# Zeudon/sound-event-localization-detection

Hardware: AMD Instinct MI355X
Metric: training clips/sec (4ch FOA 60s@24kHz) (higher is better)
Workload: dtype bf16; 1 GPU; crnn FOA 4-ch 60s clips, bs=32 windows (BASELINE configs[1]); parallelism=dp1

## Files before the change

include/seld_hip.h:

```cpp
#ifndef SELD_HIP_H_
#define SELD_HIP_H_

#include <stdint.h>

#ifdef __cplusplus
extern "C" {
#endif

int seld_init(int device);
int seld_shutdown(void);
int seld_version(void);
const char* seld_last_error(void);

int seld_set_mel_filterbank(const float* fb_host);

int seld_set_window(const float* window_host);

int seld_default_tables(float* window960, float* fb481x64, int* mel_b0_64, float* mel_wd_24x64,
                        float* mel_wu_24x64);

int64_t seld_num_frames(int64_t L);

int seld_logmel_f32(const float* pcm, int64_t N, int64_t C, int64_t L, float* out, int layout, void* stream);
int seld_logmel_i16(const int16_t* pcm, int64_t N, int64_t C, int64_t L, float* out, int layout, void* stream);
// ... 106 lines not shown
                  float* loss_out4, void* grad, void* workspace, void* stream);


int seld_gru_fold_bias(const float* b_ih, const float* b_hh, int64_t H, void* gi_bias, int out_is_bf16, float* b_hn,
                       void* stream);

int seld_gru_prepare(const float* b_ih, const float* b_hh, const void* w_hh, int w_is_bf16, int64_t H, void* gi_bias,
                     int out_is_bf16, float* b_hn, void* w_hh_t_bf16, void* stream);

int seld_gru_bias_grads(const float* partial, int64_t tiles, int64_t H, float* db_ih, float* db_hh, void* stream);

int seld_sum_chunks(const void* partial, int in_is_bf16, int64_t chunks, int64_t count, void* out, int out_is_bf16,
                    void* stream);

int64_t seld_column_sums_blocks(int64_t rows, int64_t n_cols);
int seld_column_sums(const void* g, int in_is_bf16, int64_t rows, int64_t n_cols, float* partial, void* out, int out_is_bf16,
                     void* stream);

int seld_multi_sum_chunks(const void* const* partial, void* const* out, const int64_t* counts, const int32_t* chunks,
                          const int32_t* flags, int count, void* stream);
int seld_multi_column_sums_scratch(const int64_t* rows, const int64_t* n_cols, int count, int64_t* partial_floats);
int seld_multi_column_sums(const void* const* g, void* const* out, const int64_t* rows, const int64_t* n_cols,
                           const int32_t* flags, int count, float* partial, int64_t partial_floats, void* stream);

int seld_gru_dwhh_finish(const void* p_gi, const void* p_n, int in_is_bf16, int64_t chunks, int64_t H, void* dw_hh,
                         int out_is_bf16, void* stream);

int seld_conv_weight_flip_transpose(const void* w, int elem_bytes, int64_t O, int64_t I, void* wt, void* stream);

int seld_conv3x3_wgrad_supported(int64_t F, int64_t Cin, int64_t Cout);
int64_t seld_conv3x3_wgrad_workspace_floats(int64_t B, int64_t T, int64_t F, int64_t Cin, int64_t Cout);
int seld_conv3x3_wgrad(const void* x, const void* dy, int64_t B, int64_t T, int64_t F, int64_t Cin, int64_t Cout,
                       void* dw, int dw_is_bf16, float* workspace, void* stream);

int seld_convfirst_supported(int64_t F, int64_t Cin, int64_t Cout);
int64_t seld_convfirst_workspace_floats(int backward);
int seld_convfirst_forward(const void* in, const void* w, int w_is_bf16, int64_t w_sco, int64_t w_sci, int64_t w_sr,
                           int64_t w_ss, int64_t B, int64_t T, int64_t F, const float* bn_weight, const float* bn_bias,
                           float* running_mean, float* running_var, float momentum, float eps, void* y,
                           float* mean_invstd, float* scale_shift, float* workspace, int phases, void* stream);
int seld_convfirst_backward(const void* in, const void* w, int w_is_bf16, int64_t w_sco, int64_t w_sci, int64_t w_sr,
                            int64_t w_ss, const void* dy, int64_t B, int64_t T, int64_t F, const float* mean_invstd,
                            const float* scale_shift, void* dw, int dw_is_bf16, int64_t dw_sco, int64_t dw_sci,
                            int64_t dw_sr, int64_t dw_ss, float* dgamma, float* dbeta, float* workspace, int phases,
                            void* stream);

int64_t seld_conv_tail_workspace_floats(int C);
int seld_conv_tail_forward(const void* x, const void* residual, int is_bf16, int64_t rows, int C, int pool,
                           const float* weight, const float* bias, float* running_mean, float* running_var,
                           float momentum, float eps, int training, void* y, float* mean_invstd, float* scale_shift,
                           float* workspace, void* stream);
int seld_conv_tail_backward(const void* x, const void* residual, const void* dy, int is_bf16, int64_t rows, int C,
                            int pool, const float* mean_invstd, const float* scale_shift, void* dx, void* dresidual,
                            float* dweight, float* dbias, float* workspace, void* stream);

int seld_dwconv1d(const void* x, int is_bf16, const float* weight, const float* bias, int64_t B, int64_t T, int D, int K,
                  int flip_taps, void* y, void* stream);
int64_t seld_dwconv1d_wgrad_rows(int64_t B, int64_t T);
int seld_dwconv1d_wgrad(const void* x, const void* dy, int is_bf16, int64_t B, int64_t T, int D, int K, float* partial,
                        void* stream);

int64_t seld_gru_tile_rows(void);
int seld_gru_forward(const void* gi, int is_bf16, const void* w_hh_bf16, const float* b_hn, int64_t B,
                     int64_t T, int64_t H, void* y, void* saved_tile, void* stream);

int seld_gru_backward(const void* dy_tile, const void* saved_tile, const void* y, int is_bf16,
// ... 36 lines not shown
```

sound-event-localization-detection_amd/config.py:

```python
from pathlib import Path

_SR = 24000


class Config:
    BASE_PATH = Path(__file__).parent
    AUDIO_PATH = BASE_PATH / "foa_dev"
    METADATA_PATH = BASE_PATH / "metadata_dev"
    OUTPUT_PATH = BASE_PATH / "outputs"
    CHECKPOINT_PATH = BASE_PATH / "checkpoints"

    USE_FULL_DATASET = True
    TRAIN_AUDIO_FILE = "fold3_room21_mix001.wav"
    TRAIN_META_FILE = "fold3_room21_mix001.csv"
    TEST_AUDIO_FILE = "fold4_room23_mix001.wav"
    TEST_META_FILE = "fold4_room23_mix001.csv"

    STARSS22_CLASSES = dict(enumerate((
        "Female speech, woman speaking", "Male speech, man speaking", "Clapping", "Telephone",
        "Laughter", "Domestic sounds", "Walk, footsteps", "Door, open or close", "Music",
        "Musical instrument", "Water tap, faucet", "Bell", "Knock", "Background")))

    MODEL_TYPE = "resnet_conformer"
    NUM_CLASSES = 14
# ... 21 lines not shown
    LR_DECAY_FACTOR = 0.5
    LR_DECAY_PATIENCE = 5
    WEIGHT_DECAY = 1e-4

    LOSS_TYPE = "mse"
    W_CLASS = 1.0
    W_AIUR = 1.0
    W_CL = 1.0

    PATIENCE = 20
    MIN_DELTA = 1e-4

    SAVE_EVERY_N_EPOCHS = 5
    KEEP_LAST_N_CHECKPOINTS = 3

    SPECTROGRAM_N_FFT = int(0.04 * _SR)
    SPECTROGRAM_HOP_LENGTH = int(0.02 * _SR)
    N_MELS = 64
    SR = _SR

    WINDOW_LENGTH = int(5 * _SR)
    HOP_LENGTH = int(1 * _SR)

    I = None
    J = None
    GRID_CELL_DEGREES = 10

    AMP_DTYPE = "bf16"
    CHANNELS_LAST = True
    FUSED_LOSS = True
    FUSED_CONV_TAIL = True
    CONV_DGRAD_AS_FORWARD = True
    FUSED_CONV_WGRAD = True
    FUSED_FIRST_BLOCK = True
    FUSED_DWCONV = "auto"
    CONV1X1_AS_GEMM = True
    FUSED_QKV = True
    FUSED_LAYERNORM = True
    OVERLAP_WEIGHT_GRADS = True
    FUSED_GRU = True
    DEVICE_FEED = True
    MASTER_WEIGHTS = True
    FUSED_ADAM_KERNEL = True
    GRAPH_STEP = True
    OVERLAP_ALLREDUCE = True
    ALLREDUCE_CUT_LEVELS = 2
    GRAD_REDUCE_DTYPE = "param"
    TUNED_GEMMS = True
    DDP_BUCKET_MB = 8
    SYNC_BATCHNORM = False
    SEED = None
    FEATURE_SET = "logmel"
    FEATURE_CACHE_DIR = None
    THREE_TERM_LOSS = False
    GAUSSIAN_AUGMENT = False
    GAUSSIAN_SIGMA_AZIMUTH = 5.0
    GAUSSIAN_SIGMA_ELEVATION = 5.0
    AUGMENT_SPATIAL = False
    AUGMENT_TIME_MASKS = 0
    AUGMENT_TIME_MASK_MAX = 0
    AUGMENT_FREQ_MASKS = 0
    AUGMENT_FREQ_MASK_MAX = 0
    AUGMENT_MASK_VALUE = 0.0
    FOA_CHANNEL_ORDER = "WYZX"
    GRAD_CLIP_NORM = 0.0
    SKIP_NONFINITE_STEPS = False
# ... 25 lines not shown
```

sound-event-localization-detection_amd/csrc/convwgrad.hip:

```cpp
#include <hip/hip_bf16.h>

#include "seld_common.h"

namespace seld {

namespace {

typedef __attribute__((ext_vector_type(8))) __bf16 bf16x8;
typedef __attribute__((ext_vector_type(4))) short s16x4;
typedef __attribute__((ext_vector_type(8))) short s16x8;
typedef __attribute__((ext_vector_type(4))) float f32x4;
typedef __attribute__((address_space(3))) s16x4 lds_s16x4;

constexpr int kWgThreads = 256;
constexpr int kWgTile = 64;
constexpr int kWgKc = 128;
constexpr int kWgPitch = 80;
constexpr int kWgSumThreads = 256;
constexpr int kWgSumRows = 8;

template <int F>
struct WgradGeom {
  static_assert(F == 8 || F == 16 || F == 32, "frequency bins: 8, 16 or 32");
  static constexpr int TC = kWgKc / F;
  static constexpr int XR = (TC + 2) * (F + 2);
  static constexpr int kDyLoads = kWgKc * 8 / kWgThreads;
  static constexpr int kXLoads = (XR * 8 + kWgThreads - 1) / kWgThreads;
  static constexpr int kLdsShorts = (kWgKc + XR) * kWgPitch;
  static_assert(kLdsShorts * 2 <= 64 * 1024, "LDS image larger than the default limit");
};

template <int F>
__device__ __forceinline__ int x_row(int pos) {
  return (pos / F + 1) * (F + 2) + pos % F + 1;
}

__device__ __forceinline__ s16x4 tr_read(const unsigned short* base, int offset_shorts) {
  return __builtin_amdgcn_ds_read_tr16_b64_v4i16((lds_s16x4*)(base + offset_shorts));
}

__device__ __forceinline__ bf16x8 join(s16x4 lo, s16x4 hi) {
  const s16x8 v = __builtin_shufflevector(lo, hi, 0, 1, 2, 3, 4, 5, 6, 7);
  return __builtin_bit_cast(bf16x8, v);
}

template <int F>
__global__ __launch_bounds__(kWgThreads, 2) void conv3x3_wgrad_kernel(
    const unsigned short* __restrict__ x, const unsigned short* __restrict__ dy, int T, int Cin, int Cout,
    int chunks_per_clip, int chunks, int per_slab, float* __restrict__ ws) {
  using G = WgradGeom<F>;
  __shared__ __attribute__((aligned(16))) unsigned short lds[G::kLdsShorts];
  unsigned short* const ldy = lds;
  unsigned short* const lx = lds + kWgKc * kWgPitch;

  const int tid = threadIdx.x, lane = tid & 63, wave = tid >> 6;
  const int wm = wave >> 1, wn = wave & 1;
  const int ci0 = blockIdx.x * kWgTile, co0 = blockIdx.y * kWgTile;
  const int c_begin = blockIdx.z * per_slab;
  const int c_end = min(c_begin + per_slab, chunks);

  f32x4 acc[9][2][2];
#pragma unroll
  for (int k = 0; k < 9; ++k)
#pragma unroll
    for (int m = 0; m < 2; ++m)
#pragma unroll
      for (int n = 0; n < 2; ++n) acc[k][m][n] = f32x4{0.0f, 0.0f, 0.0f, 0.0f};

  const int g = lane >> 4, q = (lane >> 2) & 3, p = lane & 3;
  const int lpos = 4 * g + q;
  const int a_col = wm * 32 + 4 * p, b_col = wn * 32 + 4 * p;

  uint4 rdy[G::kDyLoads], rx[G::kXLoads];
  auto load = [&](int c) {
    const int b = c / chunks_per_clip, t0 = (c - b * chunks_per_clip) * G::TC;
    const long clip_row = static_cast<long>(b) * T;
#pragma unroll
    for (int i = 0; i < G::kDyLoads; ++i) {
      const int piece = tid + i * kWgThreads, pos = piece >> 3, ch = piece & 7;
      const int t = t0 + pos / F;
      rdy[i] = make_uint4(0u, 0u, 0u, 0u);
      if (t < T)
        rdy[i] = *reinterpret_cast<const uint4*>(dy + ((clip_row + t) * F + pos % F) * Cout + co0 + ch * 8);
    }
#pragma unroll
    for (int i = 0; i < G::kXLoads; ++i) {
      const int piece = tid + i * kWgThreads, r = piece >> 3, ch = piece & 7;
      const int tr = r / (F + 2), f = r - tr * (F + 2) - 1, t = t0 - 1 + tr;
      rx[i] = make_uint4(0u, 0u, 0u, 0u);
      if (r < G::XR && t >= 0 && t < T && f >= 0 && f < F)
        rx[i] = *reinterpret_cast<const uint4*>(x + ((clip_row + t) * F + f) * Cin + ci0 + ch * 8);
    }
  };

  for (int c = c_begin; c < c_end; ++c) {
    load(c);
    __syncthreads();
#pragma unroll
    for (int i = 0; i < G::kDyLoads; ++i) {
      const int piece = tid + i * kWgThreads;
      *reinterpret_cast<uint4*>(ldy + (piece >> 3) * kWgPitch + (piece & 7) * 8) = rdy[i];
    }
#pragma unroll
    for (int i = 0; i < G::kXLoads; ++i) {
      const int piece = tid + i * kWgThreads;
      if (piece < G::XR * 8) *reinterpret_cast<uint4*>(lx + (piece >> 3) * kWgPitch + (piece & 7) * 8) = rx[i];
    }
    __syncthreads();

#pragma unroll
    for (int ks = 0; ks < kWgKc / 32; ++ks) {
      const int pos_lo = ks * 32 + lpos, pos_hi = pos_lo + 16;
      bf16x8 a[2];
#pragma unroll
      for (int m = 0; m < 2; ++m)
        a[m] = join(tr_read(ldy, pos_lo * kWgPitch + a_col + m * 16), tr_read(ldy, pos_hi * kWgPitch + a_col + m * 16));
      const int xr_lo = x_row<F>(pos_lo), xr_hi = x_row<F>(pos_hi);
#pragma unroll
      for (int tap = 0; tap < 9; ++tap) {
        const int shift = (tap / 3 - 1) * (F + 2) + (tap % 3 - 1);
        bf16x8 bfr[2];
#pragma unroll
        for (int n = 0; n < 2; ++n)
          bfr[n] = join(tr_read(lx, (xr_lo + shift) * kWgPitch + b_col + n * 16),
                        tr_read(lx, (xr_hi + shift) * kWgPitch + b_col + n * 16));
#pragma unroll
        for (int m = 0; m < 2; ++m)
#pragma unroll
          for (int n = 0; n < 2; ++n)
            acc[tap][m][n] = __builtin_amdgcn_mfma_f32_16x16x32_bf16(a[m], bfr[n], acc[tap][m][n], 0, 0, 0);
      }
    }
  }

  float* const slot = ws + static_cast<long>(blockIdx.z) * Cout * 9 * Cin;
#pragma unroll
  for (int m = 0; m < 2; ++m)
#pragma unroll
    for (int j = 0; j < 4; ++j) {
      const int co = co0 + wm * 32 + m * 16 + 4 * (lane >> 4) + j;
#pragma unroll
      for (int tap = 0; tap < 9; ++tap)
#pragma unroll
        for (int n = 0; n < 2; ++n)
          slot[(static_cast<long>(co) * 9 + tap) * Cin + ci0 + wn * 32 + n * 16 + (lane & 15)] = acc[tap][m][n][j];
    }
}

template <bool kBf16>
__global__ __launch_bounds__(kWgSumThreads) void conv3x3_wgrad_sum_kernel(const float* __restrict__ ws, int slabs,
                                                                           long count, void* __restrict__ dw) {
  constexpr int kCols = kWgSumThreads / kWgSumRows;
  __shared__ float4 part[kWgSumRows][kCols];
// ... 115 lines not shown
```

sound-event-localization-detection_amd/model_crnn.py:

```python
import torch
import torch.nn as nn
import torch.nn.functional as F

from seld_layernorm import run_head
from seld_linear import SeldLinear
from seld_rnn import SeldGRU


class _Conv3x3(torch.autograd.Function):

    enabled = True
    fused_wgrad = True

    @staticmethod
    def forward(ctx, x, weight):
        cdt = torch.get_autocast_dtype("cuda") if torch.is_autocast_enabled() else x.dtype
        with torch.autocast(device_type="cuda", enabled=False):
            xc, wc = x.to(cdt), weight.to(cdt)
            y = F.conv2d(xc, wc, padding=1)
        ctx.save_for_backward(xc, wc)
        ctx.dtypes = (x.dtype, weight.dtype)
        ctx.after_cut = bool(x.is_leaf and x.requires_grad)
        return y

    @staticmethod
    def backward(ctx, dy):
        xc, wc = ctx.saved_tensors
        x_dtype, w_dtype = ctx.dtypes
        with torch.autocast(device_type="cuda", enabled=False):
            dy = dy.to(xc.dtype).contiguous(memory_format=torch.channels_last)
            dx = None
            if ctx.needs_input_grad[0]:
                if wc.is_contiguous(memory_format=torch.channels_last):
                    import seld_native
                    wt = seld_native.conv_weight_flip_transpose(wc)
                else:
                    wt = wc.transpose(0, 1).flip(2, 3).contiguous(memory_format=torch.channels_last)
                import seld_overlap
                seld_overlap.release_held(dy.device)
                dx = F.conv2d(dy, wt, padding=1)
                if dx.dtype != x_dtype:
                    dx = dx.to(x_dtype)
            import seld_overlap
            import seld_native
            fused = _Conv3x3.fused_wgrad and seld_native.conv3x3_wgrad_applicable(xc, dy, wc)
            if seld_overlap.conv_wgrad_side and seld_overlap.enabled:
                dw = torch.empty_like(wc, dtype=w_dtype)

                def job():
                    if fused:
                        seld_native.conv3x3_wgrad(xc, dy, dw)
                        return
                    dw.copy_(torch.ops.aten.convolution_backward(dy, xc, wc, None, (1, 1), (1, 1), (1, 1), False, (0, 0),
                                                                 1, (False, True, False))[1])
                seld_overlap.launch_now(dy.device, [dy, xc, wc, dw], job, last_of_stage=ctx.after_cut, outputs=[dw], hold=True)
                return dx, dw.view_as(dw)
            if fused:
                return dx, seld_native.conv3x3_wgrad(xc, dy, torch.empty_like(wc, dtype=w_dtype))
            dw = torch.ops.aten.convolution_backward(dy, xc, wc, None, (1, 1), (1, 1), (1, 1), False, (0, 0), 1,
                                                     (False, True, False))[1]
        return dx, dw if dw.dtype == w_dtype else dw.to(w_dtype)


def conv3x3(c, x):
    if (x.is_cuda and _Conv3x3.enabled and c.kernel_size == (3, 3) and c.stride == (1, 1) and c.padding == (1, 1)
            and c.dilation == (1, 1) and c.groups == 1 and c.bias is None and c.padding_mode == "zeros"
            and x.is_contiguous(memory_format=torch.channels_last) and torch.is_grad_enabled()
            and (x.requires_grad or c.weight.requires_grad)):
        return _Conv3x3.apply(x, c.weight)
    return c(x)


class ConvBlock(nn.Module):
# ... 96 lines not shown
```

sound-event-localization-detection_amd/seld_native.py:

```python
from __future__ import annotations

import ctypes
import os
import threading
from pathlib import Path

import torch

_HERE = Path(__file__).resolve().parent
LIB_PATH = Path(os.environ["SELD_HIP_LIB"]).resolve() if os.environ.get("SELD_HIP_LIB") else _HERE / "libseld_hip.so"

N_FFT = 960
HOP = 480
N_BINS = 481
N_MELS = 64

_lock = threading.Lock()
_lib = None
_initialised_devices = set()

_i64 = ctypes.c_int64
_int = ctypes.c_int
_ptr = ctypes.c_void_p

# ... 41 lines not shown
    lib.seld_softmax_mse_workspace_bytes.restype = _i64
    lib.seld_softmax_mse_workspace_bytes.argtypes = []
    lib.seld_softmax_mse.argtypes = [_ptr, _int, _ptr, _ptr, _i64, _int, ctypes.c_float, _ptr, _ptr, _ptr, _ptr]
    lib.seld_scale_by_device_scalar.argtypes = [_ptr, _int, _i64, _ptr, _ptr]
    lib.seld_smr_loss_workspace_bytes.restype = _i64
    lib.seld_smr_loss_workspace_bytes.argtypes = [_i64, _i64]
    lib.seld_smr_loss.argtypes = [_ptr, _int, _ptr, _ptr, _i64, _int, _int, _int, ctypes.c_float, ctypes.c_float,
                                  ctypes.c_float, _ptr, _ptr, _ptr, _ptr]
    lib.seld_multi_cast.argtypes = [_ptr, _ptr, _ptr, _int, _int, _ptr]
    lib.seld_stream_delay.argtypes = [_i64, _ptr]
    lib.seld_gru_fold_bias.argtypes = [_ptr, _ptr, _i64, _ptr, _int, _ptr, _ptr]
    lib.seld_gru_prepare.argtypes = [_ptr, _ptr, _ptr, _int, _i64, _ptr, _int, _ptr, _ptr, _ptr]
    lib.seld_gru_bias_grads.argtypes = [_ptr, _i64, _i64, _ptr, _ptr, _ptr]
    lib.seld_sum_chunks.argtypes = [_ptr, _int, _i64, _i64, _ptr, _int, _ptr]
    lib.seld_gru_dwhh_finish.argtypes = [_ptr, _ptr, _int, _i64, _i64, _ptr, _int, _ptr]
    lib.seld_column_sums.argtypes = [_ptr, _int, _i64, _i64, _ptr, _ptr, _int, _ptr]
    _pp, _pi64, _pi32 = ctypes.POINTER(ctypes.c_void_p), ctypes.POINTER(ctypes.c_int64), ctypes.POINTER(ctypes.c_int32)
    _f = ctypes.c_float
    lib.seld_multi_adam.argtypes = [_pp, _pi32, _pp, _pp, _pp, _pp, _pi64, _int, _ptr, _ptr, _f, _f, _f, _f, _f, _ptr]
    lib.seld_multi_grad_norm_scratch.argtypes = [_pi64, _int, _pi64]
    lib.seld_multi_grad_norm.argtypes = [_pp, _pi32, _pi64, _int, _f, _f, _int, _ptr, _i64, _ptr, _ptr]
    lib.seld_multi_adam_guarded.argtypes = [_pp, _pi32, _pp, _pp, _pp, _pp, _pi64, _int, _ptr, _ptr, _f, _f, _f, _f, _f, _pp, _f,
                                            _ptr, _ptr]
    lib.seld_multi_sum_chunks.argtypes = [_pp, _pp, _pi64, _pi32, _pi32, _int, _ptr]
    lib.seld_multi_column_sums_scratch.argtypes = [_pi64, _pi64, _int, _pi64]
    lib.seld_multi_column_sums.argtypes = [_pp, _pp, _pi64, _pi64, _pi32, _int, _ptr, _i64, _ptr]
    lib.seld_column_sums_blocks.argtypes = [_i64, _i64]
    lib.seld_column_sums_blocks.restype = ctypes.c_int64
    lib.seld_conv_weight_flip_transpose.argtypes = [_ptr, _int, _i64, _i64, _ptr, _ptr]
    lib.seld_conv3x3_wgrad_supported.argtypes = [_i64, _i64, _i64]
    lib.seld_conv3x3_wgrad_workspace_floats.restype = _i64
    lib.seld_conv3x3_wgrad_workspace_floats.argtypes = [_i64, _i64, _i64, _i64, _i64]
    lib.seld_conv3x3_wgrad.argtypes = [_ptr, _ptr, _i64, _i64, _i64, _i64, _i64, _ptr, _int, _ptr, _ptr]
    lib.seld_convfirst_supported.argtypes = [_i64, _i64, _i64]
    lib.seld_convfirst_workspace_floats.restype = _i64
    lib.seld_convfirst_workspace_floats.argtypes = [_int]
    lib.seld_convfirst_forward.argtypes = [_ptr, _ptr, _int, _i64, _i64, _i64, _i64, _i64, _i64, _i64, _ptr, _ptr, _ptr, _ptr,
                                           ctypes.c_float, ctypes.c_float, _ptr, _ptr, _ptr, _ptr, _int, _ptr]
    lib.seld_convfirst_backward.argtypes = [_ptr, _ptr, _int, _i64, _i64, _i64, _i64, _ptr, _i64, _i64, _i64, _ptr, _ptr,
                                            _ptr, _int, _i64, _i64, _i64, _i64, _ptr, _ptr, _ptr, _int, _ptr]
    lib.seld_layernorm_supported.argtypes = [_i64]
    lib.seld_layernorm_workspace_floats.restype = _i64
    lib.seld_layernorm_workspace_floats.argtypes = [_i64, _i64]
    lib.seld_layernorm_forward.argtypes = [_ptr, _int, _i64, _i64, _ptr, _ptr, ctypes.c_float, _int, _ptr, _ptr, _ptr]
    lib.seld_layernorm_backward.argtypes = [_ptr, _ptr, _int, _i64, _i64, _ptr, _ptr, _ptr, _int, _ptr, _ptr, _ptr,
                                            _ptr, _ptr]
    lib.seld_conv_tail_workspace_floats.restype = _i64
    lib.seld_conv_tail_workspace_floats.argtypes = [_int]
    lib.seld_conv_tail_forward.argtypes = [_ptr, _ptr, _int, _i64, _int, _int, _ptr, _ptr, _ptr, _ptr, ctypes.c_float,
                                           ctypes.c_float, _int, _ptr, _ptr, _ptr, _ptr, _ptr]
    lib.seld_conv_tail_backward.argtypes = [_ptr, _ptr, _ptr, _int, _i64, _int, _int, _ptr, _ptr, _ptr, _ptr, _ptr, _ptr,
                                            _ptr, _ptr]
    lib.seld_dwconv1d.argtypes = [_ptr, _int, _ptr, _ptr, _i64, _i64, _int, _int, _int, _ptr, _ptr]
    lib.seld_dwconv1d_wgrad.argtypes = [_ptr, _ptr, _int, _i64, _i64, _int, _int, _ptr, _ptr]
    lib.seld_dwconv1d_wgrad_rows.argtypes = [_i64, _i64]
    lib.seld_dwconv1d_wgrad_rows.restype = ctypes.c_int64
    lib.seld_gru_to_tile.argtypes = [_ptr, _int, _i64, _i64, _int, _ptr, _ptr]
    lib.seld_gru_from_pair_tile.argtypes = [_ptr, _int, _i64, _i64, _ptr, _ptr, _ptr]
    lib.seld_gru_previous_state.argtypes = [_ptr, _int, _i64, _i64, _ptr, _ptr]
    lib.seld_gru_tile_rows.restype = _i64
    lib.seld_gru_tile_rows.argtypes = []
    lib.seld_gru_forward.argtypes = [_ptr, _int, _ptr, _ptr, _i64, _i64, _i64, _ptr, _ptr, _ptr]
    lib.seld_gru_backward.argtypes = [_ptr, _ptr, _ptr, _int, _ptr, _i64, _i64, _i64, _ptr, _ptr, _ptr]
    lib.seld_gru_backward_direct.argtypes = [_ptr, _ptr, _ptr, _int, _ptr, _i64, _i64, _i64, _ptr, _ptr, _ptr, _ptr]
    lib.seld_grid_decode.argtypes = [_ptr, _int, _i64, _i64, _i64, _i64, _ptr, _ptr, _i64, _i64, ctypes.c_float, _int,
                                     _ptr, _ptr, _ptr, _ptr, _ptr]
# ... 1014 lines not shown
    with _device_guard(ensure_init(w.device)):
        check(load_library().seld_conv_weight_flip_transpose(_p(w), w.element_size(), o, i, _p(wt),
                                                             _stream_ptr(w.device)), "seld_conv_weight_flip_transpose")
    return wt


def conv3x3_wgrad_applicable(x: torch.Tensor, dy: torch.Tensor, w: torch.Tensor) -> bool:
    if not (x.is_cuda and x.dim() == 4 and dy.dim() == 4 and w.dim() == 4 and x.dtype == torch.bfloat16
            and dy.dtype == torch.bfloat16 and tuple(w.shape[2:]) == (3, 3)):
        return False
    b, cin, t, f = x.shape
    if tuple(dy.shape) != (b, w.shape[0], t, f) or w.shape[1] != cin:
        return False
    if not (x.is_contiguous(memory_format=torch.channels_last) and dy.is_contiguous(memory_format=torch.channels_last)
            and w.is_contiguous(memory_format=torch.channels_last)):
        return False
    return bool(load_library().seld_conv3x3_wgrad_supported(f, cin, w.shape[0]))


def conv3x3_wgrad(x: torch.Tensor, dy: torch.Tensor, dw: torch.Tensor) -> torch.Tensor:
    if not conv3x3_wgrad_applicable(x, dy, dw) or dw.dtype not in (torch.float32, torch.bfloat16):
        raise SeldNativeError("conv3x3_wgrad: unsupported shapes, dtypes or layouts")
    b, cin, t, f = x.shape
    cout = dy.shape[1]
    with _device_guard(ensure_init(x.device)):
        lib = load_library()
        ws = torch.empty(int(lib.seld_conv3x3_wgrad_workspace_floats(b, t, f, cin, cout)), dtype=torch.float32,
                         device=x.device)
        check(lib.seld_conv3x3_wgrad(_p(x), _p(dy), b, t, f, cin, cout, _p(dw), _is_bf16(dw), _p(ws),
                                     _stream_ptr(x.device)), "seld_conv3x3_wgrad")
    return dw



def convfirst_applicable(x: torch.Tensor, w: torch.Tensor) -> bool:
    if not (x.is_cuda and x.dim() == 4 and w.dim() == 4 and x.dtype == torch.bfloat16
            and w.dtype in (torch.float32, torch.bfloat16) and tuple(w.shape[2:]) == (3, 3) and w.shape[1] == x.shape[1]
            and x.is_contiguous(memory_format=torch.channels_last)):
        return False
    return bool(load_library().seld_convfirst_supported(x.shape[3], x.shape[1], w.shape[0]))


def convfirst_forward(x, w, bn_weight, bn_bias, running_mean, running_var, momentum, eps, phases=3):
    if not convfirst_applicable(x, w):
        raise SeldNativeError("convfirst: unsupported shapes, dtypes or layouts")
    b, _, t, f = x.shape
    index = ensure_init(x.device)
    y = torch.empty((b, w.shape[0], t, f // 2), dtype=x.dtype, device=x.device, memory_format=torch.channels_last)
    stats = torch.empty((2, 2, w.shape[0]), dtype=torch.float32, device=x.device)
    lib = load_library()
    ws = torch.empty(int(lib.seld_convfirst_workspace_floats(0)), dtype=torch.float32, device=x.device)
    with _device_guard(index):
        check(lib.seld_convfirst_forward(_p(x), _p(w), _is_bf16(w), *w.stride(), b, t, f, _p(bn_weight), _p(bn_bias),
                                         _p(running_mean), _p(running_var), float(momentum), float(eps), _p(y),
                                         _p(stats[0]), _p(stats[1]), _p(ws), int(phases), _stream_ptr(x.device)),
              "seld_convfirst_forward")
    return y, stats[0], stats[1]


def convfirst_backward(x, w, dy, mean_invstd, scale_shift, dw, phases=3):
    if not convfirst_applicable(x, w) or dw.shape != w.shape or dw.dtype not in (torch.float32, torch.bfloat16):
        raise SeldNativeError("convfirst: unsupported shapes, dtypes or layouts")
    b, _, t, f = x.shape
    if tuple(dy.shape) != (b, w.shape[0], t, f // 2):
        raise SeldNativeError("convfirst: dy does not match the block's output")
    if dy.dtype != x.dtype or not dy.is_contiguous(memory_format=torch.channels_last):
# ... 84 lines not shown
```

sound-event-localization-detection_amd/trainer.py:

```python
import gc
import logging
import math
import os
import random
from contextlib import nullcontext
from datetime import datetime
from pathlib import Path

import numpy as np
import torch
import torch.distributed as dist
from torch.utils.data import DataLoader, RandomSampler, SequentialSampler
from tqdm import tqdm

import seld_augment
from config import Config
from dataset import SELDDataset
from loss import SMRSELDLoss
from model import SMRSELDWithCSPDarkNet
from model_conformer import SELD_Conformer
from model_crnn import SELD_CRNN
from resnet50_model import SELD_ResNet50_Conformer
from seld_rnn import SeldGRU
from utils import get_local_rank, get_rank, get_world_size, safe_torch_load
# ... 13 lines not shown
        return SELD_CRNN(n_mels=config.N_MELS, cnn_channels=config.CRNN_CNN_CHANNELS,
                         rnn_hidden=config.CRNN_RNN_HIDDEN, rnn_layers=config.CRNN_RNN_LAYERS,
                         dropout=config.CRNN_DROPOUT, **common)
    if kind == "conformer":
        logger.info("Initializing Conformer model...")
        return SELD_Conformer(n_mels=config.N_MELS, cnn_channels=config.CRNN_CNN_CHANNELS,
                              conf_d_model=config.CONF_D_MODEL, conf_n_heads=config.CONF_N_HEADS,
                              conf_n_layers=config.CONF_N_LAYERS, conf_kernel_size=config.CONF_KERNEL_SIZE,
                              dropout=config.CONF_DROPOUT, **common)
    if kind == "resnet_conformer":
        logger.info("Initializing ResNet50-Conformer model...")
        return SELD_ResNet50_Conformer(n_mels=config.N_MELS, conf_d_model=config.RESNET_CONF_D_MODEL,
                                       conf_n_heads=config.RESNET_CONF_N_HEADS,
                                       conf_n_layers=config.RESNET_CONF_N_LAYERS,
                                       dropout=config.RESNET_DROPOUT, **common)
    logger.info("Initializing CSPDarkNet (CNN) model...")
    return SMRSELDWithCSPDarkNet(use_small=use_small_model, **common)


def prepare_model_for_device(model, device):
    model = model.to(device)
    if device.type == "cuda" and getattr(config, "CHANNELS_LAST", True):
        model = model.to(memory_format=torch.channels_last)
    SeldGRU.fused_enabled = bool(getattr(config, "FUSED_GRU", True))
    if device.type == "cuda":
        import seld_convtail
        import seld_gru
        seld_convtail.enabled = bool(getattr(config, "FUSED_CONV_TAIL", True))
        import model_crnn
        model_crnn._Conv3x3.enabled = bool(getattr(config, "CONV_DGRAD_AS_FORWARD", True)) and \
            os.environ.get("SELD_CONV_AS_FWD", "1") != "0"
        model_crnn._Conv3x3.fused_wgrad = bool(getattr(config, "FUSED_CONV_WGRAD", True)) and \
            os.environ.get("SELD_CONV_WGRAD", "1") != "0"
        import seld_convfirst
        seld_convfirst.enabled = bool(getattr(config, "FUSED_FIRST_BLOCK", True)) and \
            os.environ.get("SELD_FIRST_BLOCK", "1") != "0"
        if os.environ.get("SELD_DWCONV") is None:
            import seld_dwconv
            seld_dwconv.enabled = getattr(config, "FUSED_DWCONV", "auto")
            if seld_dwconv.enabled == "auto" and graph_step_enabled(device):
                seld_dwconv.enabled = True
        import seld_layernorm
        seld_layernorm.enabled = bool(getattr(config, "FUSED_LAYERNORM", True)) and \
            os.environ.get("SELD_LAYERNORM", "1") != "0"
        if os.environ.get("SELD_OVERLAP") is None:
            import seld_overlap
            seld_overlap.enabled = bool(getattr(config, "OVERLAP_WEIGHT_GRADS", True))
        import seld_linear
        seld_linear.conv1x1_as_gemm = bool(getattr(config, "CONV1X1_AS_GEMM", True)) and \
            os.environ.get("SELD_CONV1X1_GEMM", "1") != "0"
        import model_conformer
        model_conformer.MultiHeadSelfAttention.fused_qkv = bool(getattr(config, "FUSED_QKV", True)) and \
            os.environ.get("SELD_FUSED_QKV", "1") != "0"
        for module in model.modules():
            if isinstance(module, SeldGRU) and SeldGRU.fused_enabled:
                seld_gru.pack_parameters(module)
            if isinstance(module, model_conformer.MultiHeadSelfAttention):
                module.pack_parameters()
        if os.environ.get("SELD_CUT_LEVELS") is None:
            import seld_cut
            seld_cut.levels = int(getattr(config, "ALLREDUCE_CUT_LEVELS", 2))
        import seld_tuned
        seld_tuned.enable(device, bool(getattr(config, "TUNED_GEMMS", True)))
    SMRSELDLoss.fused_enabled = bool(getattr(config, "FUSED_LOSS", True))
    return model

# ... 895 lines not shown
```

Baseline: 163.8 clips/s.

## Add fused MFMA conv3x3 data-gradient kernel reading unflipped weights directly

Adds a HIP implicit-GEMM kernel for the 3x3 convolution input gradient. It stages a padded dy image tile and weight slices in LDS and accumulates bf16 MFMA products per tap, using the negated tap shift instead of a flipped, transposed weight copy. This replaces the flip-transpose kernel plus the library conv2d call in the backward pass. Shared image-tiling helpers are moved into a common header used by the wgrad kernel too. It risks being slower than the tuned library convolution for some channel counts, and it rounds output to bf16 directly.

```diff
diff --git a/include/seld_hip.h b/include/seld_hip.h
--- a/include/seld_hip.h
+++ b/include/seld_hip.h
@@ -162,6 +162,10 @@
 int64_t seld_conv3x3_wgrad_workspace_floats(int64_t B, int64_t T, int64_t F, int64_t Cin, int64_t Cout);
 int seld_conv3x3_wgrad(const void* x, const void* dy, int64_t B, int64_t T, int64_t F, int64_t Cin, int64_t Cout,
                        void* dw, int dw_is_bf16, float* workspace, void* stream);
+
+int seld_conv3x3_dgrad_supported(int64_t F, int64_t Cin, int64_t Cout);
+int seld_conv3x3_dgrad(const void* dy, const void* w, int64_t B, int64_t T, int64_t F, int64_t Cin, int64_t Cout,
+                       void* dx, void* stream);
 
 int seld_convfirst_supported(int64_t F, int64_t Cin, int64_t Cout);
 int64_t seld_convfirst_workspace_floats(int backward);
diff --git a/sound-event-localization-detection_amd/config.py b/sound-event-localization-detection_amd/config.py
--- a/sound-event-localization-detection_amd/config.py
+++ b/sound-event-localization-detection_amd/config.py
@@ -77,6 +77,7 @@
     FUSED_CONV_TAIL = True
     CONV_DGRAD_AS_FORWARD = True
     FUSED_CONV_WGRAD = True
+    FUSED_CONV_DGRAD = True
     FUSED_FIRST_BLOCK = True
     FUSED_DWCONV = "auto"
     CONV1X1_AS_GEMM = True
diff --git a/sound-event-localization-detection_amd/csrc/conv3x3_image.h b/sound-event-localization-detection_amd/csrc/conv3x3_image.h
--- /dev/null
+++ b/sound-event-localization-detection_amd/csrc/conv3x3_image.h
@@ -0,0 +1,58 @@
+#pragma once
+
+#include <hip/hip_runtime.h>
+
+namespace seld {
+namespace conv3x3 {
+
+typedef __attribute__((ext_vector_type(8))) __bf16 bf16x8;
+typedef __attribute__((ext_vector_type(4))) short s16x4;
+typedef __attribute__((ext_vector_type(8))) short s16x8;
+typedef __attribute__((ext_vector_type(4))) float f32x4;
+typedef __attribute__((address_space(3))) s16x4 lds_s16x4;
+
+constexpr int kThreads = 256;
+constexpr int kChannels = 64;
+constexpr int kPitch = 80;
+
+template <int F, int P>
+struct Image {
+  static_assert(F == 8 || F == 16 || F == 32, "frequency bins: 8, 16 or 32");
+  static_assert(P % F == 0, "a chunk is whole time rows");
+  static constexpr int TC = P / F;
+  static constexpr int kRows = (TC + 2) * (F + 2);
+  static constexpr int kLoads = (kRows * 8 + kThreads - 1) / kThreads;
+};
+
+template <int F>
+__device__ __forceinline__ int image_row(int pos) {
+  return (pos / F + 1) * (F + 2) + pos % F + 1;
+}
+
+template <int F>
+__device__ __forceinline__ constexpr int tap_shift(int tap) {
+  return (tap / 3 - 1) * (F + 2) + (tap % 3 - 1);
+}
+
+template <int F, int P>
+__device__ __forceinline__ uint4 image_piece(const unsigned short* __restrict__ src, long clip_row, int t0, int T,
+                                             int C, int c0, int piece) {
+  const int r = piece >> 3, ch = piece & 7;
+  const int tr = r / (F + 2), f = r - tr * (F + 2) - 1, t = t0 - 1 + tr;
+  uint4 v = make_uint4(0u, 0u, 0u, 0u);
+  if (r < Image<F, P>::kRows && t >= 0 && t < T && f >= 0 && f < F)
+    v = *reinterpret_cast<const uint4*>(src + ((clip_row + t) * F + f) * C + c0 + ch * 8);
+  return v;
+}
+
+__device__ __forceinline__ s16x4 tr_read(const unsigned short* base, int offset_shorts) {
+  return __builtin_amdgcn_ds_read_tr16_b64_v4i16((lds_s16x4*)(base + offset_shorts));
+}
+
+__device__ __forceinline__ bf16x8 join(s16x4 lo, s16x4 hi) {
+  const s16x8 v = __builtin_shufflevector(lo, hi, 0, 1, 2, 3, 4, 5, 6, 7);
+  return __builtin_bit_cast(bf16x8, v);
+}
+
+}
+}
diff --git a/sound-event-localization-detection_amd/csrc/convdgrad.hip b/sound-event-localization-detection_amd/csrc/convdgrad.hip
--- /dev/null
+++ b/sound-event-localization-detection_amd/csrc/convdgrad.hip
@@ -0,0 +1,201 @@
+#include <hip/hip_bf16.h>
+
+#include "conv3x3_image.h"
+#include "seld_common.h"
+
+namespace seld {
+
+namespace {
+
+using namespace conv3x3;
+
+constexpr int kDgP = 256;
+constexpr int kDgKc = kChannels;
+
+template <int F, int NT>
+struct DgradGeom {
+  static_assert(NT == 64 || NT == 128, "input channels per workgroup: 64 or 128");
+  using Img = Image<F, kDgP>;
+  static constexpr int kWPitch = NT + 16;
+  static constexpr int kWLoads = kDgKc * NT / 8 / kThreads;
+  static constexpr int kNTiles = NT / 32;
+  static constexpr int kImgBatch = (Img::kLoads + 1) / 2;
+  static constexpr int kImgShorts = Img::kRows * kPitch;
+  static constexpr int kLdsShorts = kImgShorts + kDgKc * kWPitch;
+  static_assert(2 * kLdsShorts * 2 <= 160 * 1024, "two workgroups per CU");
+};
+
+template <int F, int NT>
+__global__ __launch_bounds__(kThreads, 2) void conv3x3_dgrad_kernel(
+    const unsigned short* __restrict__ dy, const unsigned short* __restrict__ w, int T, int Cin, int Cout,
+    int chunks_per_clip, unsigned short* __restrict__ dx) {
+  using G = DgradGeom<F, NT>;
+  __shared__ __attribute__((aligned(16))) unsigned short lds[G::kLdsShorts];
+  unsigned short* const limg = lds;
+  unsigned short* const lw = lds + G::kImgShorts;
+
+  const int tid = threadIdx.x, lane = tid & 63, wave = tid >> 6;
+  const int wm = wave >> 1, wn = wave & 1;
+  const int chunk = blockIdx.x, ci0 = blockIdx.y * NT;
+  const int b = chunk / chunks_per_clip, t0 = (chunk - b * chunks_per_clip) * G::Img::TC;
+  const long clip_row = static_cast<long>(b) * T;
+
+  f32x4 acc[8][G::kNTiles];
+#pragma unroll
+  for (int m = 0; m < 8; ++m)
+#pragma unroll
+    for (int n = 0; n < G::kNTiles; ++n) acc[m][n] = f32x4{0.0f, 0.0f, 0.0f, 0.0f};
+
+  const int g = lane >> 4, q = (lane >> 2) & 3, p = lane & 3, l15 = lane & 15;
+  const int w_off = (4 * g + q) * G::kWPitch + wn * (NT / 2) + 4 * p;
+  const int d_off = image_row<F>(wm * 128 + l15) * kPitch + 8 * g;
+  auto d_rows = [](int m) { return image_row<F>(16 * m) - image_row<F>(0); };
+
+  static_assert(G::kWLoads == 2 || G::kWLoads == 4, "weight pieces per thread");
+  uint4 rw0, rw1, rw2 = make_uint4(0u, 0u, 0u, 0u), rw3 = rw2;
+  auto w_piece = [&](int stage, int i) {
+    const int kc = stage / 9, tap = stage - kc * 9;
+    const int piece = tid + i * kThreads, row = piece / (NT / 8), ch = piece % (NT / 8);
+    return *reinterpret_cast<const uint4*>(w + (static_cast<long>(kc * kDgKc + row) * 9 + tap) * Cin + ci0 + ch * 8);
+  };
+  auto load_w = [&](int stage) {
+    rw0 = w_piece(stage, 0);
+    rw1 = w_piece(stage, 1);
+    if constexpr (G::kWLoads == 4) {
+      rw2 = w_piece(stage, 2);
+      rw3 = w_piece(stage, 3);
+    }
+  };
+  auto w_slot = [&](int i) {
+    const int piece = tid + i * kThreads;
+    return reinterpret_cast<uint4*>(lw + piece / (NT / 8) * G::kWPitch + piece % (NT / 8) * 8);
+  };
+
+  const int stages = Cout / kDgKc * 9;
+  load_w(0);
+  for (int stage = 0; stage < stages; ++stage) {
+    const int kc = stage / 9, tap = stage - kc * 9;
+    uint4 rimg[G::kImgBatch];
+    auto load_img = [&](int first) {
+#pragma unroll
+      for (int i = 0; i < G::kImgBatch; ++i)
+        rimg[i] = image_piece<F, kDgP>(dy, clip_row, t0, T, Cout, kc * kDgKc, tid + (first + i) * kThreads);
+    };
+    auto store_img = [&](int first) {
+#pragma unroll
+      for (int i = 0; i < G::kImgBatch; ++i) {
+        const int piece = tid + (first + i) * kThreads, ch = piece & 7;
+        unsigned short* const dst = limg + (piece >> 3) * kPitch + (ch >> 2) * 32 + 16 * (ch & 1) + 4 * ((ch >> 1) & 1);
+        if (piece < G::Img::kRows * 8) {
+          *reinterpret_cast<uint2*>(dst) = make_uint2(rimg[i].x, rimg[i].y);
+          *reinterpret_cast<uint2*>(dst + 8) = make_uint2(rimg[i].z, rimg[i].w);
+        }
+      }
+    };
+    if (tap == 0) load_img(0);
+    __syncthreads();
+    *w_slot(0) = rw0;
+    *w_slot(1) = rw1;
+    if constexpr (G::kWLoads == 4) {
+      *w_slot(2) = rw2;
+      *w_slot(3) = rw3;
+    }
+    if (tap == 0) {
+      store_img(0);
+      load_img(G::kImgBatch);
+      store_img(G::kImgBatch);
+    }
+    __syncthreads();
+    load_w(min(stage + 1, stages - 1));
+
+    const int shift = -tap_shift<F>(tap) * kPitch;
+#pragma unroll
+    for (int ks = 0; ks < kDgKc / 32; ++ks) {
+      bf16x8 wf[G::kNTiles];
+#pragma unroll
+      for (int n = 0; n < G::kNTiles; ++n)
+        wf[n] = join(tr_read(lw, w_off + ks * 32 * G::kWPitch + n * 16),
+                     tr_read(lw, w_off + (ks * 32 + 16) * G::kWPitch + n * 16));
+#pragma unroll
+      for (int m = 0; m < 8; ++m) {
+        const bf16x8 df = *reinterpret_cast<const bf16x8*>(limg + d_off + d_rows(m) * kPitch + shift + ks * 32);
+#pragma unroll
+        for (int n = 0; n < G::kNTiles; ++n)
+          acc[m][n] = __builtin_amdgcn_mfma_f32_16x16x32_bf16(wf[n], df, acc[m][n], 0, 0, 0);
+      }
+    }
+  }
+
+  const int rows_left = (T - t0) * F;
+  unsigned short* const out = dx + ((clip_row + t0) * F) * Cin + ci0 + wn * (NT / 2) + 4 * g;
+#pragma unroll
+  for (int m = 0; m < 8; ++m) {
+    const int pos = wm * 128 + m * 16 + l15;
+    if (pos >= rows_left) continue;
+#pragma unroll
+    for (int n = 0; n < G::kNTiles; ++n) {
+      const f32x4 v = acc[m][n];
+      const unsigned lo = static_cast<unsigned>(__bfloat16_as_ushort(__float2bfloat16(v[0]))) |
+                          (static_cast<unsigned>(__bfloat16_as_ushort(__float2bfloat16(v[1]))) << 16);
+      const unsigned hi = static_cast<unsigned>(__bfloat16_as_ushort(__float2bfloat16(v[2]))) |
+                          (static_cast<unsigned>(__bfloat16_as_ushort(__float2bfloat16(v[3]))) << 16);
+      *reinterpret_cast<uint2*>(out + static_cast<long>(pos) * Cin + n * 16) = make_uint2(lo, hi);
+    }
+  }
+}
+
+bool dgrad_supported(int64_t F, int64_t Cin, int64_t Cout) {
+  return (F == 8 || F == 16 || F == 32) && Cin > 0 && Cout > 0 && Cin % 64 == 0 && Cout % kDgKc == 0;
+}
+
+template <int F>
+void launch_dgrad(const unsigned short* dy, const unsigned short* w, int B, int T, int Cin, int Cout,
+                  unsigned short* dx, hipStream_t stream) {
+  constexpr int tc = kDgP / F;
+  const int chunks_per_clip = (T + tc - 1) / tc;
+  const unsigned chunks = static_cast<unsigned>(B * chunks_per_clip);
+  if (Cin % 128 == 0)
+    hipLaunchKernelGGL((conv3x3_dgrad_kernel<F, 128>), dim3(chunks, static_cast<unsigned>(Cin / 128)), dim3(kThreads),
+                       0, stream, dy, w, T, Cin, Cout, chunks_per_clip, dx);
+  else
+    hipLaunchKernelGGL((conv3x3_dgrad_kernel<F, 64>), dim3(chunks, static_cast<unsigned>(Cin / 64)), dim3(kThreads), 0,
+                       stream, dy, w, T, Cin, Cout, chunks_per_clip, dx);
+}
+
+}
+
+}
+
+extern "C" {
+
+int seld_conv3x3_dgrad_supported(int64_t F, int64_t Cin, int64_t Cout) {
+  return seld::dgrad_supported(F, Cin, Cout) ? 1 : 0;
+}
+
+int seld_conv3x3_dgrad(const void* dy, const void* w, int64_t B, int64_t T, int64_t F, int64_t Cin, int64_t Cout,
+                       void* dx, void* stream_) {
+  using namespace seld;
+  const DeviceState* st = current_state();
+  if (!st) return kErrNotInitialised;
+  if (!dy || !w || !dx || B <= 0 || T <= 0) return fail(kErrInvalidArgument, "seld_conv3x3_dgrad: bad argument");
+  if (!dgrad_supported(F, Cin, Cout))
+    return fail(kErrUnsupported, "seld_conv3x3_dgrad: F in {8, 16, 32} and channel counts % 64 == 0 required");
+  if (B * ((T + kDgP / F - 1) / (kDgP / F)) > 0x7fffffffLL || B * T > 0x7fffffffLL)
+    return fail(kErrUnsupported, "seld_conv3x3_dgrad: too many positions");
+  if (((reinterpret_cast<uintptr_t>(dy) | reinterpret_cast<uintptr_t>(w) | reinterpret_cast<uintptr_t>(dx)) & 15) != 0)
+    return fail(kErrInvalidArgument, "seld_conv3x3_dgrad: 16-byte aligned tensors required");
+  hipStream_t stream = static_cast<hipStream_t>(stream_);
+  const unsigned short* ds = static_cast<const unsigned short*>(dy);
+  const unsigned short* ws = static_cast<const unsigned short*>(w);
+  unsigned short* xs = static_cast<unsigned short*>(dx);
+  const int b = static_cast<int>(B), t = static_cast<int>(T), ci = static_cast<int>(Cin), co = static_cast<int>(Cout);
+  switch (F) {
+    case 8: launch_dgrad<8>(ds, ws, b, t, ci, co, xs, stream); break;
+    case 16: launch_dgrad<16>(ds, ws, b, t, ci, co, xs, stream); break;
+    default: launch_dgrad<32>(ds, ws, b, t, ci, co, xs, stream); break;
+  }
+  SELD_HIP_TRY(hipGetLastError());
+  return kOk;
+}
+
+}
diff --git a/sound-event-localization-detection_amd/csrc/convwgrad.hip b/sound-event-localization-detection_amd/csrc/convwgrad.hip
--- a/sound-event-localization-detection_amd/csrc/convwgrad.hip
+++ b/sound-event-localization-detection_amd/csrc/convwgrad.hip
@@ -1,48 +1,31 @@
 #include <hip/hip_bf16.h>
 
+#include "conv3x3_image.h"
 #include "seld_common.h"
 
 namespace seld {
 
 namespace {
 
-typedef __attribute__((ext_vector_type(8))) __bf16 bf16x8;
-typedef __attribute__((ext_vector_type(4))) short s16x4;
-typedef __attribute__((ext_vector_type(8))) short s16x8;
-typedef __attribute__((ext_vector_type(4))) float f32x4;
-typedef __attribute__((address_space(3))) s16x4 lds_s16x4;
-
-constexpr int kWgThreads = 256;
+using namespace conv3x3;
+
+constexpr int kWgThreads = kThreads;
 constexpr int kWgTile = 64;
 constexpr int kWgKc = 128;
-constexpr int kWgPitch = 80;
+constexpr int kWgPitch = kPitch;
 constexpr int kWgSumThreads = 256;
 constexpr int kWgSumRows = 8;
 
 template <int F>
 struct WgradGeom {
-  static_assert(F == 8 || F == 16 || F == 32, "frequency bins: 8, 16 or 32");
-  static constexpr int TC = kWgKc / F;
-  static constexpr int XR = (TC + 2) * (F + 2);
+  using Img = Image<F, kWgKc>;
+  static constexpr int TC = Img::TC;
+  static constexpr int XR = Img::kRows;
   static constexpr int kDyLoads = kWgKc * 8 / kWgThreads;
-  static constexpr int kXLoads = (XR * 8 + kWgThreads - 1) / kWgThreads;
+  static constexpr int kXLoads = Img::kLoads;
   static constexpr int kLdsShorts = (kWgKc + XR) * kWgPitch;
   static_assert(kLdsShorts * 2 <= 64 * 1024, "LDS image larger than the default limit");
 };
-
-template <int F>
-__device__ __forceinline__ int x_row(int pos) {
-  return (pos / F + 1) * (F + 2) + pos % F + 1;
-}
-
-__device__ __forceinline__ s16x4 tr_read(const unsigned short* base, int offset_shorts) {
-  return __builtin_amdgcn_ds_read_tr16_b64_v4i16((lds_s16x4*)(base + offset_shorts));
-}
-
-__device__ __forceinline__ bf16x8 join(s16x4 lo, s16x4 hi) {
-  const s16x8 v = __builtin_shufflevector(lo, hi, 0, 1, 2, 3, 4, 5, 6, 7);
-  return __builtin_bit_cast(bf16x8, v);
-}
 
 template <int F>
 __global__ __launch_bounds__(kWgThreads, 2) void conv3x3_wgrad_kernel(
@@ -85,11 +68,7 @@
     }
 #pragma unroll
     for (int i = 0; i < G::kXLoads; ++i) {
-      const int piece = tid + i * kWgThreads, r = piece >> 3, ch = piece & 7;
-      const int tr = r / (F + 2), f = r - tr * (F + 2) - 1, t = t0 - 1 + tr;
-      rx[i] = make_uint4(0u, 0u, 0u, 0u);
-      if (r < G::XR && t >= 0 && t < T && f >= 0 && f < F)
-        rx[i] = *reinterpret_cast<const uint4*>(x + ((clip_row + t) * F + f) * Cin + ci0 + ch * 8);
+      rx[i] = image_piece<F, kWgKc>(x, clip_row, t0, T, Cin, ci0, tid + i * kWgThreads);
     }
   };
 
@@ -115,10 +94,10 @@
 #pragma unroll
       for (int m = 0; m < 2; ++m)
         a[m] = join(tr_read(ldy, pos_lo * kWgPitch + a_col + m * 16), tr_read(ldy, pos_hi * kWgPitch + a_col + m * 16));
-      const int xr_lo = x_row<F>(pos_lo), xr_hi = x_row<F>(pos_hi);
+      const int xr_lo = image_row<F>(pos_lo), xr_hi = image_row<F>(pos_hi);
 #pragma unroll
       for (int tap = 0; tap < 9; ++tap) {
-        const int shift = (tap / 3 - 1) * (F + 2) + (tap % 3 - 1);
+        const int shift = tap_shift<F>(tap);
         bf16x8 bfr[2];
 #pragma unroll
         for (int n = 0; n < 2; ++n)
diff --git a/sound-event-localization-detection_amd/model_crnn.py b/sound-event-localization-detection_amd/model_crnn.py
--- a/sound-event-localization-detection_amd/model_crnn.py
+++ b/sound-event-localization-detection_amd/model_crnn.py
@@ -11,6 +11,7 @@
 
     enabled = True
     fused_wgrad = True
+    fused_dgrad = True
 
     @staticmethod
     def forward(ctx, x, weight):
@@ -31,14 +32,18 @@
             dy = dy.to(xc.dtype).contiguous(memory_format=torch.channels_last)
             dx = None
             if ctx.needs_input_grad[0]:
-                if wc.is_contiguous(memory_format=torch.channels_last):
-                    import seld_native
-                    wt = seld_native.conv_weight_flip_transpose(wc)
+                import seld_native
+                import seld_overlap
+                if _Conv3x3.fused_dgrad and seld_native.conv3x3_dgrad_applicable(dy, wc):
+                    seld_overlap.release_held(dy.device)
+                    dx = seld_native.conv3x3_dgrad(dy, wc)
                 else:
-                    wt = wc.transpose(0, 1).flip(2, 3).contiguous(memory_format=torch.channels_last)
-                import seld_overlap
-                seld_overlap.release_held(dy.device)
-                dx = F.conv2d(dy, wt, padding=1)
+                    if wc.is_contiguous(memory_format=torch.channels_last):
+                        wt = seld_native.conv_weight_flip_transpose(wc)
+                    else:
+                        wt = wc.transpose(0, 1).flip(2, 3).contiguous(memory_format=torch.channels_last)
+                    seld_overlap.release_held(dy.device)
+                    dx = F.conv2d(dy, wt, padding=1)
                 if dx.dtype != x_dtype:
                     dx = dx.to(x_dtype)
             import seld_overlap
diff --git a/sound-event-localization-detection_amd/seld_native.py b/sound-event-localization-detection_amd/seld_native.py
--- a/sound-event-localization-detection_amd/seld_native.py
+++ b/sound-event-localization-detection_amd/seld_native.py
@@ -97,6 +97,8 @@
     lib.seld_conv3x3_wgrad_workspace_floats.restype = _i64
     lib.seld_conv3x3_wgrad_workspace_floats.argtypes = [_i64, _i64, _i64, _i64, _i64]
     lib.seld_conv3x3_wgrad.argtypes = [_ptr, _ptr, _i64, _i64, _i64, _i64, _i64, _ptr, _int, _ptr, _ptr]
+    lib.seld_conv3x3_dgrad_supported.argtypes = [_i64, _i64, _i64]
+    lib.seld_conv3x3_dgrad.argtypes = [_ptr, _ptr, _i64, _i64, _i64, _i64, _i64, _ptr, _ptr]
     lib.seld_convfirst_supported.argtypes = [_i64, _i64, _i64]
     lib.seld_convfirst_workspace_floats.restype = _i64
     lib.seld_convfirst_workspace_floats.argtypes = [_int]
@@ -1177,6 +1179,31 @@
     return dw
 
 
+def conv3x3_dgrad_applicable(dy: torch.Tensor, w: torch.Tensor) -> bool:
+    if not (dy.is_cuda and dy.dim() == 4 and w.dim() == 4 and dy.dtype == torch.bfloat16 and w.dtype == torch.bfloat16
+            and tuple(w.shape[2:]) == (3, 3) and dy.shape[1] == w.shape[0]):
+        return False
+    if not (dy.is_contiguous(memory_format=torch.channels_last) and w.is_contiguous(memory_format=torch.channels_last)):
+        return False
+    return bool(load_library().seld_conv3x3_dgrad_supported(dy.shape[3], w.shape[1], w.shape[0]))
+
+
+def conv3x3_dgrad(dy: torch.Tensor, w: torch.Tensor, out: "torch.Tensor | None" = None) -> torch.Tensor:
+    if not conv3x3_dgrad_applicable(dy, w):
+        raise SeldNativeError("conv3x3_dgrad: unsupported shapes, dtypes or layouts")
+    b, cout, t, f = dy.shape
+    cin = w.shape[1]
+    if out is None:
+        out = torch.empty((b, cin, t, f), dtype=torch.bfloat16, device=dy.device, memory_format=torch.channels_last)
+    elif not (out.dtype == torch.bfloat16 and out.device == dy.device and tuple(out.shape) == (b, cin, t, f)
+              and out.is_contiguous(memory_format=torch.channels_last)):
+        raise SeldNativeError("conv3x3_dgrad: out must be bf16 [B, Cin, T, F] in channels-last memory")
+    with _device_guard(ensure_init(dy.device)):
+        check(load_library().seld_conv3x3_dgrad(_p(dy), _p(w), b, t, f, cin, cout, _p(out), _stream_ptr(dy.device)),
+              "seld_conv3x3_dgrad")
+    return out
+
+
 
 def convfirst_applicable(x: torch.Tensor, w: torch.Tensor) -> bool:
     if not (x.is_cuda and x.dim() == 4 and w.dim() == 4 and x.dtype == torch.bfloat16
diff --git a/sound-event-localization-detection_amd/trainer.py b/sound-event-localization-detection_amd/trainer.py
--- a/sound-event-localization-detection_amd/trainer.py
+++ b/sound-event-localization-detection_amd/trainer.py
@@ -69,6 +69,8 @@
             os.environ.get("SELD_CONV_AS_FWD", "1") != "0"
         model_crnn._Conv3x3.fused_wgrad = bool(getattr(config, "FUSED_CONV_WGRAD", True)) and \
             os.environ.get("SELD_CONV_WGRAD", "1") != "0"
+        model_crnn._Conv3x3.fused_dgrad = bool(getattr(config, "FUSED_CONV_DGRAD", True)) and \
+            os.environ.get("SELD_CONV_DGRAD", "1") != "0"
         import seld_convfirst
         seld_convfirst.enabled = bool(getattr(config, "FUSED_FIRST_BLOCK", True)) and \
             os.environ.get("SELD_FIRST_BLOCK", "1") != "0"
```

New measurement: 167.9 clips/s (median of 6 runs). +2.5%, better.
